# kylegrover/raymarch-algo-compare

Hardware: AMD Instinct MI355X
Metric: Mrays/sec (mean iters/ray alongside), 1920x1080 Mandelbulb/Standard (higher is better)
Workload: dtype f64

## Files before the change

raymarch_algo_compare_amd/csrc/rm_core.h:

```cpp
#pragma once

#include <stdint.h>

#if defined(__HIPCC__)
#include <hip/hip_runtime.h>
#define RM_HD __host__ __device__ __forceinline__
#else
#define RM_HD inline __attribute__((always_inline))
#endif

#include "rm_math.h"

namespace rm {

RM_HD double py_max(double a, double b) { return (b > a) ? b : a; }
RM_HD double py_min(double a, double b) { return (b < a) ? b : a; }

RM_HD double py_mod_pow2(double a, double b)
{
    double m = a - rm_trunc(a / b) * b;
    if (m != 0.0) {
        if (m < 0.0) m += b;
    } else {
        m = 0.0;
// ... 7 lines not shown

RM_HD vec3 v3(double x, double y, double z)
{
    vec3 r;
    r.x = x; r.y = y; r.z = z;
    return r;
}
RM_HD vec3 operator+(vec3 a, vec3 b) { return v3(a.x + b.x, a.y + b.y, a.z + b.z); }
RM_HD vec3 operator-(vec3 a, vec3 b) { return v3(a.x - b.x, a.y - b.y, a.z - b.z); }
RM_HD vec3 operator*(vec3 a, double s) { return v3(a.x * s, a.y * s, a.z * s); }
RM_HD double dot(vec3 a, vec3 b) { return a.x * b.x + a.y * b.y + a.z * b.z; }
RM_HD double pow_half(double x) { return rm_pow(x, 0.5); }
RM_HD double length(vec3 a) { return pow_half(a.x * a.x + a.y * a.y + a.z * a.z); }
RM_HD double pow_half_a(double x) { return rm_pow_half<true>(x); }
RM_HD double length_a(vec3 a) { return pow_half_a(a.x * a.x + a.y * a.y + a.z * a.z); }
RM_HD vec3 normalized(vec3 a)
{
    double l = length(a);
    if (l < 1e-12) return v3(0.0, 0.0, 0.0);
    double inv = 1.0 / l;
    return v3(a.x * inv, a.y * inv, a.z * inv);
}

struct StratParams {
    double omega;
    double ar_omega_min;
    double ar_omega_max;
    double ar_smoothing;
    double ar_growth_rate;
    double ar_decay_rate;
// ... 40 lines not shown
```

raymarch_algo_compare_amd/csrc/rm_kernels.h:

```cpp
#pragma once

#define RM_TABLES_IN_LDS 1

#include <hip/hip_runtime.h>
#include <stdint.h>
#include <type_traits>

#include "rm_camera.h"
#include "rm_capture.h"
#include "rm_scenes.h"
#include "rm_shape.h"
#include "rm_strategies.h"

namespace rm {

constexpr int kHistBins = 544;
constexpr int kStatsHead = 24;
constexpr int kStatsWords = kStatsHead + kHistBins;
constexpr int kQueues = 2;
constexpr int kStatsParts = 64;
constexpr int kStatsBlocks = 1 + kStatsParts;

struct FrameParams {
    CameraParams cam;
// ... 687 lines not shown
    rm_load_tables<Scene>();
    size_t i = (size_t)blockIdx.x * blockDim.x + threadIdx.x;
    if (i >= n) return;
    vec3 o = v3(origins[3 * i], origins[3 * i + 1], origins[3 * i + 2]);
    vec3 d = normalized(v3(dirs[3 * i], dirs[3 * i + 1], dirs[3 * i + 2]));
    Result r = march_one<Scene, Strat>(o, d, cfg);
    hit[i] = (uint8_t)r.hit; t[i] = r.t; iters[i] = r.iters; final_sdf[i] = r.final_sdf;
}

constexpr int kTeam = 3;

struct TeamXch {
    double v[2][2 * kTeam][64];
};

template <class Scene, class PartT>
__device__ __forceinline__ bool team_trip(typename Scene::Eval& ev, bool go, PartT part, int lane, TeamXch& x, int& turn)
{
    double o0 = 0.0, o1 = 0.0;
    if constexpr (std::is_same<PartT, int>::value) {
        if (go) Scene::trip_part(ev, part, o0, o1);
    } else {
        if (go) Scene::template trip_part<PartT::value>(ev, o0, o1);
    }
    double (*buf)[64] = x.v[turn & 1];
    ++turn;
    buf[2 * (int)part][lane] = o0;
    buf[2 * (int)part + 1][lane] = o1;
    __syncthreads();
    bool done = true;
    if (go) done = Scene::trip_join(ev, buf[0][lane], buf[1][lane], buf[2][lane], buf[3][lane], buf[4][lane], buf[5][lane]);
    return done;
}

template <class Scene, class = void>
struct ScenePartLoops : std::false_type {};
template <class Scene>
struct ScenePartLoops<Scene, decltype((void)Scene::kPartLoops)> : std::integral_constant<bool, Scene::kPartLoops> {};

template <class Scene, class = void>
struct SceneShortLastTrip : std::false_type {};
template <class Scene>
struct SceneShortLastTrip<Scene, decltype((void)Scene::kLastTrip)> : std::true_type {};

template <class Scene, int P, class Trip>
__device__ __forceinline__ void team_trips_part(bool& ready, const Trip& trip)
{
    if constexpr (SceneShortLastTrip<Scene>::value) {
#pragma unroll 1
        for (int n = 0; n < Scene::kLastTrip && __any(!ready); ++n) {
            const bool fin = trip(std::integral_constant<int, P>(), !ready);
            if (!ready) ready = fin;
        }
    } else {
        while (__any(!ready)) {
            const bool fin = trip(std::integral_constant<int, P>(), !ready);
            if (!ready) ready = fin;
        }
    }
}
template <class Scene, class Trip>
__device__ __forceinline__ void team_trips(int part, bool& ready, typename Scene::Eval& ev, const Trip& trip)
{
    if constexpr (ScenePartLoops<Scene>::value) {
        part = __builtin_amdgcn_readfirstlane(part);
        if (part == 0) team_trips_part<Scene, 0>(ready, trip);
        else if (part == 1) team_trips_part<Scene, 1>(ready, trip);
        else team_trips_part<Scene, 2>(ready, trip);
        if constexpr (SceneShortLastTrip<Scene>::value) {
            if (__any(!ready)) {
                if (!ready) Scene::trip_last(ev);
                ready = true;
            }
        }
    } else {
        static_assert(!SceneShortLastTrip<Scene>::value, "the short last trip is built into the per-part loops only");
        while (__any(!ready)) {
            const bool fin = trip(part, !ready);
            if (!ready) ready = fin;
        }
    }
}

// ... 13 lines not shown
    const int lane = lane_id();
    const int part = (int)(threadIdx.x >> 6);
    const size_t i = (size_t)blockIdx.x * 64 + (size_t)lane;
    const bool have = i < n;
    vec3 o = v3(0.0, 0.0, 0.0), d = v3(0.0, 0.0, 1.0);
    if (have) {
        o = v3(origins[3 * i], origins[3 * i + 1], origins[3 * i + 2]);
        d = normalized(v3(dirs[3 * i], dirs[3 * i + 1], dirs[3 * i + 2]));
    }
    Strat s;
    bool done = true;
    if (have) done = s.start(cfg);
    typename Scene::Eval ev;
    int turn = 0;
    while (__any(!done)) {
        bool ready = true;
        if (!done) ready = Scene::begin(ev, o + d * s.te);
        team_trips<Scene>(part, ready, ev, [&](auto P, bool go) { return team_trip<Scene>(ev, go, P, lane, xch, turn); });
        if (!done) done = s.step(Scene::value(ev), cfg);
    }
    if (have && part == 0) {
        hit[i] = (uint8_t)s.res.hit; t[i] = s.res.t; iters[i] = s.res.iters; final_sdf[i] = s.res.final_sdf;
    }
    if (busy && threadIdx.x == 0) __hip_atomic_fetch_add(busy, 1ull, __ATOMIC_RELAXED, __HIP_MEMORY_SCOPE_AGENT);
}

template <class Scene, class Strat, bool BATCH>
__global__ __launch_bounds__(64 * kTeam) void resume_team_kernel(const KernelArgs a, const int level)
{
    using Entry = QEntry<Strat>;
    __shared__ TeamXch xch;
    __shared__ unsigned int s_hist[kHistBins];
    __shared__ unsigned int s_base;
// ... 60 lines not shown
                        lane_cfg.full = a.full;
                    } else {
                        camera_ray(a.single.cam, a.width, a.height, x, gy, origin, dir);
                    }
                    active = true;
                }
            }
        }
        if (!__any(active)) {
            if (!more) break;
            continue;
        }

        bool ready = true;
        if (active) ready = Scene::begin(ev, origin + dir * s.te);
        team_trips<Scene>(part, ready, ev, [&](auto P, bool go) { return team_trip<Scene>(ev, go, P, lane, xch, turn); });
        bool park = false;
        if (active) {
            ++nev;
            if (!s.step(Scene::value(ev), cfg)) {
                park = a.suspend_after > 0 && s.i >= a.suspend_after;
            } else {
            active = false;
            if (part == 0) {
                const int it = s.res.iters, h = s.res.hit;
                a.depth[my_gi] = h ? (float)s.res.t : 0.0f;
                a.iters[my_gi] = it;
                a.hit[my_gi] = (uint8_t)h;
                if (raw_out) store_raw(a, my_gi, s.res, nev);
                acc.evals += (unsigned)nev;
                acc.add(it, h);
// ... 113 lines not shown
```

raymarch_algo_compare_amd/csrc/rm_math_atan.h:

```cpp
#pragma once

namespace rm {

struct AtanK {
    static constexpr double hpi = 0x1.921fb54442d18p+0, hpi1 = 0x1.1a62633145c07p-54;
    static constexpr double opi = 0x1.921fb54442d18p+1, opi1 = 0x1.1a62633145c07p-53;
    static constexpr double d3 = -0x1.5555555555555p-2, d5 = 0x1.99999999997fdp-3, d7 = -0x1.24924923f7603p-3,
                            d9 = 0x1.c71c6e5129a3bp-4, d11 = -0x1.7458022b13c25p-4, d13 = 0x1.375f08b31cbcep-4;
    static constexpr double f1 = 0x1.55555555554f9p-3, f2 = 0x1.333333336127dp-4, f3 = 0x1.6db6dae42c0e4p-5,
                            f4 = 0x1.f1c7e04f4ad99p-6, f5 = 0x1.6e442c822d419p-6, f6 = 0x1.292d80f453c72p-6;
    static constexpr double rt0 = 0x1.fffffffecc1ddp-1, rt1 = 0x1.fffffff757304p-2, rt2 = 0x1.800496769c91ap-2,
                            rt3 = 0x1.4006318d1dab9p-2;
    static constexpr double t27 = 0x1p27;
};


RM_MATH_HD double rm_acos_sqrt_band(double x, int m)
{
    typedef AtanK K;
    const double zp = 1.0 - x, zn = x + 1.0;
    double z = ((m > 0) ? zp : zn) * 0.5;
    const int kz = (int)(rm_asuint64(z) >> 32);
    double t = rm_inroot[(kz >> 14) & 0x7f] * rm_asdouble((uint64_t)((1023 + 511 - (kz >> 21)) & 0x7ff) << 52);
    double r = rm_fnma(t * t, z, 1.0);
// ... 6 lines not shown
    double y = rm_fnma(K::t27, c, rm_fma(c, K::t27, c));
    double ty = rm_fma(h, c, y);
    double cc = rm_fnma(y, y, z) / ty;
    double p = rm_fma(z, K::f6, K::f5);
    p = rm_fma(z, p, K::f4);
    p = rm_fma(z, p, K::f3);
    p = rm_fma(z, p, K::f2);
    p = rm_fma(z, p, K::f1);
    double pz = (p * z) * (y + cc);
    const double res_neg = ((K::hpi1 - cc) - pz) + (K::hpi - y);
    const double res_pos = (cc + pz) + y;
    const double res = (m < 0) ? res_neg : res_pos;
    return res + res;
}

RM_MATH_HD double rm_acos_team(double x)
{
    typedef AtanK K;
    const uint64_t bits = rm_asuint64(x);
    const int m = (int)(bits >> 32);
    const int k = m & 0x7fffffff;
    const bool pos = m > 0;
    const double ax = rm_fabs(x);
    const bool in_taylor = k < 0x3fc00000, in_sqrt = k >= 0x3fef0000;
    const bool any_special = rm_band_needed<true>((k < 0x3c880000) | (k >= 0x3ff00000));

    double res = 0.0;
    if (rm_band_needed<true>(!in_taylor & !in_sqrt)) {
        const int r1 = (k >> 15) & 0x1f, r2 = 32 + ((k >> 14) & 0x3f), r3 = 96 + ((k >> 13) & 0x7f);
        int row = (k >= 0x3fd00000) ? r2 : r1;
        row = (k >= 0x3fe00000) ? r3 : row;
// ... 29 lines not shown
    }
    if (rm_band_needed<true>(in_sqrt & (k < 0x3ff00000))) {
        const double res_sqrt = rm_acos_sqrt_band(x, m);
        res = in_sqrt ? res_sqrt : res;
    }
    if (any_special) {
        res = (k < 0x3c880000) ? K::hpi : res;
        const double at_one = pos ? 0.0 : K::opi;
        const bool is_one = (k == 0x3ff00000) & ((uint32_t)bits == 0);
        const double beyond = is_one ? at_one : __builtin_nan("");
        res = (k >= 0x3ff00000) ? beyond : res;
    }
    return res;
}

template <bool U = false>
RM_MATH_HD double rm_acos(double x)
{
    typedef AtanK K;
    if constexpr (U) return rm_acos_team(x);
    const uint64_t bits = rm_asuint64(x);
    const int m = (int)(bits >> 32);
    const int k = m & 0x7fffffff;
    const bool pos = m > 0;
    const double ax = rm_fabs(x);

    double res_taylor = 0.0;
    if (rm_band_needed<U>(k < 0x3fc00000)) {
        const double x2 = x * x;
        double pt = rm_fma(x2, K::f6, K::f5);
        pt = rm_fma(x2, pt, K::f4);
        pt = rm_fma(x2, pt, K::f3);
        pt = rm_fma(x2, pt, K::f2);
        pt = rm_fma(x2, pt, K::f1);
        const double rt = K::hpi - x;
// ... 36 lines not shown
    res = (k >= 0x3ff00000) ? beyond : res;
    return res;
}


RM_MATH_HD double rm_atan_series(double v)
{
    typedef AtanK K;
    double p = rm_fma(v, K::d13, K::d11);
    p = rm_fma(v, p, K::d9);
    p = rm_fma(v, p, K::d7);
    p = rm_fma(v, p, K::d5);
    return rm_fma(v, p, K::d3);
}

RM_MATH_HD double rm_atan2_team(double y, double x)
{
    typedef AtanK K;
    const uint32_t ux = (uint32_t)(rm_asuint64(x) >> 32), uy = (uint32_t)(rm_asuint64(y) >> 32);
    const int de = (int)(uy & 0x7ff00000u) - (int)(ux & 0x7ff00000u);
    const uint32_t lo_e = (1023u - 500u) << 20, span_e = 1000u << 20;
    const bool off_path = rm_band_needed<true>((((ux & 0x7ff00000u) - lo_e) >= span_e) | (((uy & 0x7ff00000u) - lo_e) >= span_e) |
                                               ((uint32_t)(de + (56 << 20)) > (uint32_t)(112 << 20)));

    double ax = rm_fabs(x), ay = rm_fabs(y);
    if (off_path) {
        const double up = ((ax < 0x1p-500) | (ay < 0x1p-500)) ? 0x1p500 : 1.0;
        ax *= up; ay *= up;
        const double dn = ((ax > 0x1p500) | (ay > 0x1p500)) ? 0x1p-500 : 1.0;
        ax *= dn; ay *= dn;
    }
// ... 53 lines not shown
    }
    if (off_path) {
        const bool xneg = (ux & 0x80000000u) != 0;
        const double z_tiny = xpos ? u : K::opi;
        z = (de <= -59768832) ? z_tiny : z;
        z = (de >= 59768832) ? K::hpi : z;
        z = (x == 0.0) ? K::hpi : z;
        const double z_y0 = xneg ? K::opi : 0.0;
        z = (y == 0.0) ? z_y0 : z;
        const bool nonfinite = ((ux & 0x7ff00000u) == 0x7ff00000u) | ((uy & 0x7ff00000u) == 0x7ff00000u);
        z = nonfinite ? __builtin_nan("") : z;
    }
    return __builtin_copysign(z, y);
}

template <bool U = false>
RM_MATH_HD double rm_atan2(double y, double x)
{
    typedef AtanK K;
    if constexpr (U) return rm_atan2_team(y, x);
    const uint32_t ux = (uint32_t)(rm_asuint64(x) >> 32), uy = (uint32_t)(rm_asuint64(y) >> 32);
    const int de = (int)(uy & 0x7ff00000u) - (int)(ux & 0x7ff00000u);

    double ax = rm_fabs(x), ay = rm_fabs(y);
    const double up = ((ax < 0x1p-500) | (ay < 0x1p-500)) ? 0x1p500 : 1.0;
    ax *= up; ay *= up;
    const double dn = ((ax > 0x1p500) | (ay > 0x1p500)) ? 0x1p-500 : 1.0;
    ax *= dn; ay *= dn;

    const bool y_lt_x = ay < ax;
    const double num = y_lt_x ? ay : ax, den = y_lt_x ? ax : ay;
    const double u = num / den;
    const double vq = den * u;
    const double du = ((num - vq) - rm_fma(den, u, -vq)) / den;

// ... 63 lines not shown
```

raymarch_algo_compare_amd/csrc/rm_math_pow.h:

```cpp
#pragma once

#include "rm_tables.h"

namespace rm {

RM_MATH_HD uint64_t rm_asuint64(double x) { return __builtin_bit_cast(uint64_t, x); }
RM_MATH_HD double rm_asdouble(uint64_t u) { return __builtin_bit_cast(double, u); }

RM_MATH_HD double rm_pow_log_inline(uint64_t ix, double* tail)
{
    const double Ln2hi = rm_pow_log_head[0], Ln2lo = rm_pow_log_head[1];
    const double A0 = rm_pow_log_head[2], A1 = rm_pow_log_head[3], A2 = rm_pow_log_head[4],
                 A3 = rm_pow_log_head[5], A4 = rm_pow_log_head[6], A5 = rm_pow_log_head[7],
                 A6 = rm_pow_log_head[8];
    uint64_t tmp = ix - 0x3fe6955500000000ull;
    int i = (int)((tmp >> 45) & 127);
    int k = (int)((int64_t)tmp >> 52);
    uint64_t iz = ix - (tmp & 0xfff0000000000000ull);
    double z = rm_asdouble(iz);
    double kd = (double)k;
    double invc = tab_pow_log(i, 0);
    double logc = tab_pow_log(i, 1);
    double logctail = tab_pow_log(i, 2);

// ... 92 lines not shown
#if defined(__HIP_DEVICE_COMPILE__)
    if constexpr (SPARSE) {
        if (__popcll(__ballot(true)) <= kSparseLanes) {
            bool safe;
            double r = rm_pow_half_guard(x, &safe);
            if (__any(!safe)) {
                const double full = rm_pow(x, 0.5);
                r = safe ? r : full;
            }
            return r;
        }
    }
#endif
    return rm_pow(x, 0.5);
}
RM_MATH_HD void rm_pow2(double x, double ya, double yb, double* ra, double* rb)
{
    double lo;
    double hi = rm_pow_log_inline(rm_pow_norm_bits(x), &lo);
    double ehia = ya * hi, ehib = yb * hi;
    double eloa = rm_fma(ya, lo, rm_fma(hi, ya, -ehia));
    double elob = rm_fma(yb, lo, rm_fma(hi, yb, -ehib));
    *ra = rm_pow_fix_special(x, rm_pow_exp_inline(ehia, eloa));
    *rb = rm_pow_fix_special(x, rm_pow_exp_inline(ehib, elob));
}

}
```

raymarch_algo_compare_amd/csrc/rm_math_trig.h:

```cpp
#pragma once

namespace rm {


struct SinCosK {
    static constexpr double big = 0x1.8p45, toint = 0x1.8p52;
    static constexpr double hpinv = 0x1.45f306dc9c883p-1;
    static constexpr double hp0 = 0x1.921fb54442d18p+0, hp1 = 0x1.1a62633145c07p-54;
    static constexpr double mp1 = 0x1.921fb58000000p+0, mp2 = -0x1.dde973c000000p-27;
    static constexpr double pp3 = -0x1.cb3b398000000p-55, pp4 = -0x1.d747f23e32ed7p-83;
    static constexpr double sn3 = -0x1.5555555555515p-3, sn5 = 0x1.11110e829872fp-7;
    static constexpr double cs2 = 0.5, cs4 = -0x1.5555555555535p-5, cs6 = 0x1.6c16bedd9e239p-10;
    static constexpr double s1 = -0x1.5555555555555p-3, s2 = 0x1.1111111110ecep-7, s3 = -0x1.a01a019db08b8p-13,
                            s4 = 0x1.71de27b9a7ed9p-19, s5 = -0x1.addffc2fcdf59p-26;
};

RM_MATH_HD double rm_fnma(double a, double b, double c) { return rm_fma(-a, b, c); }

template <bool U>
RM_MATH_HD bool rm_band_needed(bool lane_selects)
{
#if defined(__HIP_DEVICE_COMPILE__)
    if constexpr (U) return __any(lane_selects) != 0;
#endif
    (void)lane_selects;
    return true;
}

RM_MATH_HD double rm_taylor_sin(double x, double dx)
{
    typedef SinCosK K;
    double xx = x * x;
    double p = rm_fma(xx, K::s5, K::s4);
    p = rm_fma(xx, p, K::s3);
    p = rm_fma(xx, p, K::s2);
    p = rm_fma(xx, p, K::s1);
    double q = rm_fma(p, x, -(dx * 0.5));
    double t = rm_fma(xx, q, dx);
    return x + t;
}

// ... 27 lines not shown
{
    typedef SinCosK K;
    const double aa = rm_fabs(a);
    const double dx = (a < 0.0) ? -da : da;
    const double u = K::big + aa;
    const double x = (aa - (u - K::big)) + dx;
    const int k = rm_sincos_row(u);
    const double sn = tab_sincos(k, 0), ssn = tab_sincos(k, 1), cs = tab_sincos(k, 2), ccs = tab_sincos(k, 3);
    const double xx = x * x;
    const double s = rm_fma(x * xx, rm_fma(xx, K::sn5, K::sn3), x);
    const double c = xx * rm_fma(xx, rm_fma(xx, K::cs6, K::cs4), K::cs2);
    const double cor = rm_fnma(s, sn, rm_fnma(c, cs, rm_fnma(s, ssn, ccs)));
    return cs + cor;
}

RM_MATH_HD double rm_do_sin_team(double a, double da)
{
    typedef SinCosK K;
    const double aa = rm_fabs(a);
    const double dx = (a <= 0.0) ? -da : da;
    const double u = K::big + aa;
    const double x = aa - (u - K::big);
    const int k = rm_sincos_row(u);
    const double sn = tab_sincos(k, 0), ssn = tab_sincos(k, 1), cs = tab_sincos(k, 2), ccs = tab_sincos(k, 3);
    const double xx = x * x;
    const double s = x + rm_fma(x * xx, rm_fma(xx, K::sn5, K::sn3), dx);
    const double c = rm_fma(x, dx, xx * rm_fma(xx, rm_fma(xx, K::cs6, K::cs4), K::cs2));
    const double cor = rm_fma(s, cs, rm_fnma(c, sn, rm_fma(s, ccs, ssn)));
    double res = __builtin_copysign(sn + cor, a);
    if (rm_band_needed<true>(aa < 0.126)) {
        const double taylor = rm_taylor_sin(a, da);
        res = (aa < 0.126) ? taylor : res;
    }
    return res;
}

RM_MATH_HD void rm_sincos_team(double x, double* sin_out, double* cos_out)
{
    typedef SinCosK K;
    const uint32_t k = (uint32_t)(rm_asuint64(x) >> 32) & 0x7fffffffu;
    const double ax = rm_fabs(x);
    const bool r1 = k < 0x3feb6000u;
    const bool r2 = !r1 & (k < 0x400368fdu);
    const bool any_r2 = rm_band_needed<true>(r2);
    const bool any_edge = rm_band_needed<true>(r2 | (k - 0x3e500000u >= 0x419921fbu - 0x3e500000u));
    const double t = rm_fma(x, K::hpinv, K::toint);
    const double xn = r1 ? 0.0 : (t - K::toint);
    const uint32_t n = r1 ? 0u : (uint32_t)rm_asuint64(t);
    const double y = rm_fnma(xn, K::mp2, rm_fnma(xn, K::mp1, x));
    const double t2 = rm_fnma(xn, K::pp3, y);
    double db = rm_fnma(K::pp3, xn, y - t2);
    const double b = rm_fnma(xn, K::pp4, t2);
    db = db + rm_fnma(xn, K::pp4, t2 - b);

    double aS = b, daS = db, aC = b, daC = db;
    if (any_r2) {
        const double tt = K::hp0 - ax;
        const double a2 = tt + K::hp1;
        const double da2 = (tt - a2) + K::hp1;
        aS = r2 ? a2 : b, daS = r2 ? da2 : db, aC = r2 ? tt : b, daC = r2 ? K::hp1 : db;
    }
    const double dS = rm_do_sin_team(aS, daS);
    const double dC = rm_do_cos(aC, daC);

    const uint32_t m = n + 1u;
    double s = (n & 1u) ? dC : dS;
    s = (n & 2u) ? -s : s;
    double c = (m & 1u) ? dC : dS;
    c = (m & 2u) ? -c : c;
    if (any_edge) {
        const double s2 = __builtin_copysign(dC, x);
        s = r2 ? s2 : s, c = r2 ? dS : c;
        s = (k < 0x3e500000u) ? x : s;
        c = (k < 0x3e400000u) ? 1.0 : c;
        const double bad = __builtin_nan("");
        const bool huge = k >= 0x419921fbu;
        s = huge ? bad : s;
        c = huge ? bad : c;
    }
    *sin_out = s;
    *cos_out = c;
}

template <bool U = false>
RM_MATH_HD void rm_sincos(double x, double* sin_out, double* cos_out)
{
    typedef SinCosK K;
    if constexpr (U) return rm_sincos_team(x, sin_out, cos_out);
    const uint32_t k = (uint32_t)(rm_asuint64(x) >> 32) & 0x7fffffffu;
    const double ax = rm_fabs(x);
    const bool r1 = k < 0x3feb6000u;
    const bool r2 = !r1 & (k < 0x400368fdu);
    const double t = rm_fma(x, K::hpinv, K::toint);
    const double xn = r1 ? 0.0 : (t - K::toint);
    const uint32_t n = r1 ? 0u : (uint32_t)rm_asuint64(t);
    const double y = rm_fnma(xn, K::mp2, rm_fnma(xn, K::mp1, x));
    const double t2 = rm_fnma(xn, K::pp3, y);
    double db = rm_fnma(K::pp3, xn, y - t2);
    const double b = rm_fnma(xn, K::pp4, t2);
    db = db + rm_fnma(xn, K::pp4, t2 - b);
    const double tt = K::hp0 - ax;
    const double a2 = tt + K::hp1;
    const double da2 = (tt - a2) + K::hp1;
// ... 92 lines not shown
```

raymarch_algo_compare_amd/csrc/rm_pipeline.h:

```cpp
#pragma once

#include "rm_kernels.h"

namespace rm {

constexpr int kCtlStride = 16;
constexpr int kCTile = 0;
constexpr int kCReserved = 1;
constexpr int kCTaken = 3;
constexpr int kCFreshDone = 5;
constexpr int kCProdExited = 6;
constexpr int kCLeft = 7;
constexpr int kCLateStarted = 8;
constexpr int kCTeamDone = 9;
constexpr int kCtlWords = 10 * kCtlStride;
__device__ __forceinline__ unsigned long long* ctl(const KernelArgs& a, int k) { return a.ctl + k * kCtlStride; }
constexpr int kWMarkStart = 13;
constexpr int kWMarkFresh = 14;
constexpr int kWMarkProd = 15;
constexpr int kWMarkTiles = 17;
constexpr int kWMarkPush = 18;
constexpr int kWMarkPop = 19;
constexpr int kWLongPushMax = 20;
constexpr int kWLongTeamMax = 21;
// ... 154 lines not shown
        const uint32_t y = pix / (uint32_t)a.width, x = pix - y * (uint32_t)a.width;
        atomicMax(&a.tile_cost[frame * (uint32_t)a.tiles_per_frame + (y / (uint32_t)a.tile_h) * (uint32_t)a.tiles_x + (x >> 6)], it);
    }
}

template <class Scene, class E>
__device__ __forceinline__ auto early_handover(const KernelArgs& a, const E& ev, int i) -> decltype(Scene::eval_trips(ev), bool())
{
    return a.early_handover > 0 && i >= a.early_handover && Scene::eval_trips(ev) >= a.early_trips;
}
template <class Scene>
__device__ __forceinline__ bool early_handover(const KernelArgs&, const NoEval&, int) { return false; }
template <class Scene, class E>
__device__ __forceinline__ bool early_handover(const KernelArgs&, const E&, long) { return false; }

template <class Scene, class Strat, bool BATCH>
__device__ __forceinline__ void pipe_team_role(const KernelArgs& a, const KernelArgs& ar, PipeTeamLds& L, const int part, const int lane)
{
    WaveAcc acc;
    if (a.team_prio >= 3) __builtin_amdgcn_s_setprio(3);
    else if (a.team_prio == 2) __builtin_amdgcn_s_setprio(2);
    else if (a.team_prio == 1) __builtin_amdgcn_s_setprio(1);
    bool active = false;
    uint32_t my_gi = 0;
    uint32_t my_push = 0;
    uint32_t my_pop = 0, nev_pop = 0;
    int nev = 0;
    vec3 origin = v3(0.0, 0.0, 0.0), dir = v3(0.0, 0.0, 0.0);
    MarchCfg lane_cfg = a.single.cfg;
    if constexpr (!BATCH) pin_cfg(lane_cfg);
    const MarchCfg& cfg = lane_cfg;
// ... 66 lines not shown
                        lane_cfg.full = ar.full;
                    } else {
                        camera_ray(ar.single.cam, ar.width, ar.height, x, gy, origin, dir);
                    }
                    active = true;
                }
            } else if (nidle == 64) {
                __builtin_amdgcn_s_sleep(127);
                __builtin_amdgcn_s_sleep(127);
                continue;
            }
        }
        if (!__any(active)) continue;

        ++since_try;
        bool ready = true;
        if (active) ready = Scene::begin(ev, origin + dir * s.te);
        team_trips<Scene>(part, ready, ev, [&](auto P, bool go) { return team_trip<Scene>(ev, go, P, lane, L.xch, turn); });
        const int live = a.trace ? __popcll(__ballot(active)) : 0;
        if (active) {
            ++nev;
            if (s.step(Scene::value(ev), cfg)) {
                active = false;
                if (part == 0) {
                    store_direct(ar, my_gi, s.res, nev, acc, L.hist);
                    if (ar.trace) {
                        const uint32_t k = atomicAdd(&ar.trace[0], 1u);
                        if (k < ar.trace_cap) {
                            uint32_t* const r = ar.trace + 8 + 8 * (size_t)k;
                            r[0] = my_gi; r[1] = (uint32_t)s.res.iters; r[2] = my_push; r[3] = my_pop;
                            r[4] = (uint32_t)(realtime() - ~ld_relaxed(&ar.stats[kWMarkStart]));
                            r[5] = nev_pop; r[6] = (uint32_t)nev; r[7] = (uint32_t)blockIdx.x | ((uint32_t)live << 16);
                        }
// ... 48 lines not shown
    constexpr int kRole[8] = { 0, 1, 2, -1, -1, -1, -1, -1 };
    const int wave_role = !team_wg ? -2 : kRole[wave & 7];
    const bool team_role = team_wg && wave_role >= 0;
    if (team_wg) {
        PipeTeamLds& T = *reinterpret_cast<PipeTeamLds*>(s_role);
        for (int b = threadIdx.x; b < kHistBins; b += blockDim.x) T.hist[b] = 0u;
        if (threadIdx.x == 0) { T.base = T.count = T.queue = T.done = 0u; T.ok_lo = T.ok_hi = 0u; }
        __syncthreads();
    }

    if constexpr (TEAM_ROLE) {
    if (team_wg && wave_role == -1) return;
    if (team_role) {
        const int team = wave_role / kTeam;
        const int part = wave_role % kTeam;
        pipe_team_role<Scene, Strat, BATCH>(a, a, reinterpret_cast<PipeTeamLds*>(s_role)[team], part, lane);
        return;
    }
    }

    PLds& L = *reinterpret_cast<PLds*>(s_role);
    float (*const s_depth)[TILE_PIX] = L.depth[wave];
    uint32_t (*const s_ih)[TILE_PIX] = L.ih[wave];
    const int ntiles = ka.tiles_per_frame * ka.nframes;
    const int team_wgs = TEAM_ROLE ? a.team_wgs : 0;
    int pwave = ((int)blockIdx.x - team_wgs) * kPipeWaves + wave;
    if constexpr (SPLIT) pwave = __builtin_amdgcn_readfirstlane(pwave);
    const int park0 = ka.suspend_after;
    const int park1 = (TEAMS && ka.team_wgs > 0) ? ka.suspend_after2 : 0;
    const bool queues = park0 > 0;
    const bool detach = SPLIT || a.q0_detach != 0;
// ... 369 lines not shown
    if (threadIdx.x == 0) s_args = a;
    pipeline_body<Scene, Strat, TILE_H, INTERLEAVE, BATCH, false, true>(a, s_args);
}

template <class Scene, class Strat, bool BATCH>
__global__ __launch_bounds__(64 * kTeam) void pipeline_team_kernel(const KernelArgs a)
{
    __shared__ PipeTeamLds T;
    __shared__ KernelArgs s_args;
    if (threadIdx.x == 0) s_args = a;
    for (int b = threadIdx.x; b < kHistBins; b += blockDim.x) T.hist[b] = 0u;
    if (threadIdx.x == 0) { T.base = T.count = T.queue = T.done = 0u; T.ok_lo = T.ok_hi = 0u; }
    rm_load_tables<Scene>();
    __syncthreads();
    if (a.marks && threadIdx.x == 0) atomicMax(&a.stats[kWMarkStart], ~realtime());
    pipe_team_role<Scene, Strat, BATCH>(a, s_args, T, (int)(threadIdx.x >> 6), lane_id());
}

}
```

raymarch_algo_compare_amd/csrc/rm_scenes.h:

```cpp
#pragma once

#include "rm_core.h"

namespace rm {

enum : unsigned { TB_POW = 1u, TB_SINCOS = 2u, TB_ACOS = 4u, TB_ATAN = 8u, TB_LOG = 16u };
template <class Scene> struct SceneTables { static constexpr unsigned value = TB_POW; };
template <class Scene> struct SceneIterative { static constexpr bool value = false; };


RM_HD double sd_sphere(vec3 p, double radius) { return length(p) - radius; }

RM_HD double sd_box(vec3 p, vec3 b)
{
    vec3 q = v3(rm_fabs(p.x) - b.x, rm_fabs(p.y) - b.y, rm_fabs(p.z) - b.z);
    double outside = length(v3(py_max(q.x, 0.0), py_max(q.y, 0.0), py_max(q.z, 0.0)));
    double inside = py_min(py_max(q.x, py_max(q.y, q.z)), 0.0);
    return outside + inside;
}

RM_HD double sd_plane(vec3 p, vec3 n, double offset) { return dot(p, n) - offset; }

RM_HD double sd_cylinder(vec3 p, double radius, double half_height)
{
// ... 102 lines not shown
            d = py_max(d, c);
        }
        return d;
    }
};
struct SceneMandelbulb {
    struct Eval {
        vec3 p, z;
        double dr, r;
        int32_t i;
    };
    static RM_HD bool begin(Eval& e, vec3 p)
    {
        e.p = p; e.z = p; e.dr = 1.0; e.i = 0;
        e.r = length_a(p);
        return e.r > 4.0;
    }
    static RM_HD int eval_trips(const Eval& e) { return e.i; }
    static RM_HD bool trip(Eval& e)
    {
        const double power = 8.0;
        const vec3 z = e.z;
        const double r = e.r;
        double theta = rm_acos(py_max(-1.0, py_min(1.0, z.z / py_max(r, 1e-12))));
        double phi = rm_atan2(z.y, z.x);
        double r7, zr;
        rm_pow2(r, power - 1.0, power, &r7, &zr);
        e.dr = r7 * power * e.dr + 1.0;
        theta *= power;
        phi *= power;
// ... 2 lines not shown
        rm_sincos(phi, &sp, &cp);
        e.z = v3(zr * st * cp, zr * st * sp, zr * ct) + e.p;
        if (++e.i >= 8) return true;
        e.r = length_a(e.z);
        return e.r > 4.0;
    }
    static constexpr int kLastTrip = 7;
    static RM_HD void trip_last(Eval& e)
    {
        const double power = 8.0;
        const double r7 = rm_pow(e.r, power - 1.0);
        e.dr = r7 * power * e.dr + 1.0;
        e.i = kLastTrip + 1;
    }
    static constexpr bool kPartLoops = true;
    template <int P>
    static RM_HD void trip_part(const Eval& e, double& o0, double& o1)
    {
        const double power = 8.0;
        if constexpr (P == 0) {
            double theta = rm_acos<true>(py_max(-1.0, py_min(1.0, e.z.z / py_max(e.r, 1e-12))));
            theta *= power;
            rm_sincos<true>(theta, &o0, &o1);
        } else if constexpr (P == 1) {
            double phi = rm_atan2<true>(e.z.y, e.z.x);
            phi *= power;
            rm_sincos<true>(phi, &o0, &o1);
        } else {
            rm_pow2(e.r, power - 1.0, power, &o0, &o1);
        }
    }
    static RM_HD void trip_part(const Eval& e, int part, double& o0, double& o1)
    {
        if (part == 0) trip_part<0>(e, o0, o1);
        else if (part == 1) trip_part<1>(e, o0, o1);
        else trip_part<2>(e, o0, o1);
    }
    static RM_HD bool trip_join(Eval& e, double st, double ct, double sp, double cp, double r7, double zr)
    {
        const double power = 8.0;
        e.dr = r7 * power * e.dr + 1.0;
        e.z = v3(zr * st * cp, zr * st * sp, zr * ct) + e.p;
        if (++e.i >= 8) return true;
        e.r = length_a(e.z);
        return e.r > 4.0;
    }
    static RM_HD double value(const Eval& e)
    {
        return 0.5 * rm_log(py_max(e.r, 1e-12)) * e.r / py_max(e.dr, 1e-12);
    }
    static RM_HD double sdf(vec3 p)
    {
        Eval e;
        bool done = begin(e, p);
#pragma unroll 1
        for (int i = 0; !done; ++i) {
            if (i == kLastTrip) { trip_last(e); break; }
            done = trip(e);
        }
// ... 209 lines not shown
```

Before: 288.8.

## Add common-path fast branches for team math and sparse-wave evaluation

Splits the team acos, atan2 and sincos into a common path that takes a single table branch unless a wave-wide rare check sees lanes needing the Taylor, sqrt or edge bands. It also adds a sparse-wave mode: when few lanes are live, the evaluation uses a different sqrt routine and reads the wave's own trip-part outputs from registers rather than LDS. The aim is to cut divergent band evaluation and exchange overhead in the Mandelbulb team kernels, at the cost of more code paths and template instantiations. The older banded path is kept for the non-flag pipeline role.

```diff
diff --git a/raymarch_algo_compare_amd/csrc/rm_core.h b/raymarch_algo_compare_amd/csrc/rm_core.h
--- a/raymarch_algo_compare_amd/csrc/rm_core.h
+++ b/raymarch_algo_compare_amd/csrc/rm_core.h
@@ -45,6 +45,7 @@
 RM_HD double length(vec3 a) { return pow_half(a.x * a.x + a.y * a.y + a.z * a.z); }
 RM_HD double pow_half_a(double x) { return rm_pow_half<true>(x); }
 RM_HD double length_a(vec3 a) { return pow_half_a(a.x * a.x + a.y * a.y + a.z * a.z); }
+RM_HD double length_a(vec3 a, bool sparse) { return rm_pow_half_sparse(a.x * a.x + a.y * a.y + a.z * a.z, sparse); }
 RM_HD vec3 normalized(vec3 a)
 {
     double l = length(a);
diff --git a/raymarch_algo_compare_amd/csrc/rm_kernels.h b/raymarch_algo_compare_amd/csrc/rm_kernels.h
--- a/raymarch_algo_compare_amd/csrc/rm_kernels.h
+++ b/raymarch_algo_compare_amd/csrc/rm_kernels.h
@@ -725,14 +725,45 @@
     double v[2][2 * kTeam][64];
 };
 
+template <class Scene, class = void>
+struct SceneSparseFlag : std::false_type {};
+template <class Scene>
+struct SceneSparseFlag<Scene, decltype((void)Scene::kSparseFlag)> : std::integral_constant<bool, Scene::kSparseFlag> {};
+__device__ __forceinline__ bool team_sparse(bool live) { return __popcll(__ballot(live)) <= kSparseLanes; }
+template <class Scene, int P, bool SPARSE>
+__device__ __forceinline__ bool team_trip(typename Scene::Eval& ev, bool go, int lane, TeamXch& x, int& turn)
+{
+    double o0 = 0.0, o1 = 0.0;
+    if (go) Scene::template trip_part<P, SPARSE>(ev, o0, o1);
+    double (*buf)[64] = x.v[turn & 1];
+    ++turn;
+    buf[2 * P][lane] = o0;
+    buf[2 * P + 1][lane] = o1;
+    __syncthreads();
+    bool done = true;
+    if (go) {
+        double v[2 * kTeam];
+#pragma unroll
+        for (int k = 0; k < 2 * kTeam; ++k) v[k] = (k == 2 * P) ? o0 : (k == 2 * P + 1) ? o1 : buf[k][lane];
+        done = Scene::trip_join(ev, v[0], v[1], v[2], v[3], v[4], v[5], SPARSE);
+    }
+    return done;
+}
+
+template <class Scene, int P>
+__device__ __forceinline__ void team_trip_part_banded(const typename Scene::Eval& ev, double& o0, double& o1)
+{
+    if constexpr (SceneSparseFlag<Scene>::value) Scene::template trip_part<P, false>(ev, o0, o1);
+    else Scene::template trip_part<P>(ev, o0, o1);
+}
 template <class Scene, class PartT>
-__device__ __forceinline__ bool team_trip(typename Scene::Eval& ev, bool go, PartT part, int lane, TeamXch& x, int& turn)
+__device__ __forceinline__ bool team_trip_banded(typename Scene::Eval& ev, bool go, PartT part, int lane, TeamXch& x, int& turn)
 {
     double o0 = 0.0, o1 = 0.0;
     if constexpr (std::is_same<PartT, int>::value) {
         if (go) Scene::trip_part(ev, part, o0, o1);
     } else {
-        if (go) Scene::template trip_part<PartT::value>(ev, o0, o1);
+        if (go) team_trip_part_banded<Scene, PartT::value>(ev, o0, o1);
     }
     double (*buf)[64] = x.v[turn & 1];
     ++turn;
@@ -754,8 +785,40 @@
 template <class Scene>
 struct SceneShortLastTrip<Scene, decltype((void)Scene::kLastTrip)> : std::true_type {};
 
+template <class Scene, int P, bool SPARSE>
+__device__ __forceinline__ void team_flag_trips(bool& ready, typename Scene::Eval& ev, int lane, TeamXch& x, int& turn)
+{
+#pragma unroll 1
+    for (int n = 0; n < Scene::kLastTrip && __any(!ready); ++n) {
+        const bool fin = team_trip<Scene, P, SPARSE>(ev, !ready, lane, x, turn);
+        if (!ready) ready = fin;
+    }
+}
+template <class Scene, bool SPARSE>
+__device__ __forceinline__ void team_flag_evaluation(int part, bool live, vec3 o, vec3 d, double t, typename Scene::Eval& ev, int lane,
+                                                     TeamXch& x, int& turn)
+{
+    bool ready = true;
+    if (live) ready = Scene::begin(ev, o + d * t, SPARSE);
+    if (part == 0) team_flag_trips<Scene, 0, SPARSE>(ready, ev, lane, x, turn);
+    else if (part == 1) team_flag_trips<Scene, 1, SPARSE>(ready, ev, lane, x, turn);
+    else team_flag_trips<Scene, 2, SPARSE>(ready, ev, lane, x, turn);
+    if (__any(!ready)) {
+        if (!ready) Scene::trip_last(ev);
+    }
+}
+template <class Scene>
+__device__ __forceinline__ void team_evaluate(int part, bool live, vec3 o, vec3 d, double t, typename Scene::Eval& ev, int lane, TeamXch& x,
+                                              int& turn)
+{
+    static_assert(ScenePartLoops<Scene>::value && SceneShortLastTrip<Scene>::value, "built for the Mandelbulb's loops");
+    part = __builtin_amdgcn_readfirstlane(part);
+    if (team_sparse(live)) team_flag_evaluation<Scene, true>(part, live, o, d, t, ev, lane, x, turn);
+    else team_flag_evaluation<Scene, false>(part, live, o, d, t, ev, lane, x, turn);
+}
+
 template <class Scene, int P, class Trip>
-__device__ __forceinline__ void team_trips_part(bool& ready, const Trip& trip)
+__device__ __forceinline__ void team_trips_banded_part(bool& ready, const Trip& trip)
 {
     if constexpr (SceneShortLastTrip<Scene>::value) {
 #pragma unroll 1
@@ -775,9 +838,9 @@
 {
     if constexpr (ScenePartLoops<Scene>::value) {
         part = __builtin_amdgcn_readfirstlane(part);
-        if (part == 0) team_trips_part<Scene, 0>(ready, trip);
-        else if (part == 1) team_trips_part<Scene, 1>(ready, trip);
-        else team_trips_part<Scene, 2>(ready, trip);
+        if (part == 0) team_trips_banded_part<Scene, 0>(ready, trip);
+        else if (part == 1) team_trips_banded_part<Scene, 1>(ready, trip);
+        else team_trips_banded_part<Scene, 2>(ready, trip);
         if constexpr (SceneShortLastTrip<Scene>::value) {
             if (__any(!ready)) {
                 if (!ready) Scene::trip_last(ev);
@@ -821,9 +884,13 @@
     typename Scene::Eval ev;
     int turn = 0;
     while (__any(!done)) {
-        bool ready = true;
-        if (!done) ready = Scene::begin(ev, o + d * s.te);
-        team_trips<Scene>(part, ready, ev, [&](auto P, bool go) { return team_trip<Scene>(ev, go, P, lane, xch, turn); });
+        if constexpr (SceneSparseFlag<Scene>::value) {
+            team_evaluate<Scene>(part, !done, o, d, s.te, ev, lane, xch, turn);
+        } else {
+            bool ready = true;
+            if (!done) ready = Scene::begin(ev, o + d * s.te);
+            team_trips<Scene>(part, ready, ev, [&](auto P, bool go) { return team_trip_banded<Scene>(ev, go, P, lane, xch, turn); });
+        }
         if (!done) done = s.step(Scene::value(ev), cfg);
     }
     if (have && part == 0) {
@@ -914,7 +981,7 @@
 
         bool ready = true;
         if (active) ready = Scene::begin(ev, origin + dir * s.te);
-        team_trips<Scene>(part, ready, ev, [&](auto P, bool go) { return team_trip<Scene>(ev, go, P, lane, xch, turn); });
+        team_trips<Scene>(part, ready, ev, [&](auto P, bool go) { return team_trip_banded<Scene>(ev, go, P, lane, xch, turn); });
         bool park = false;
         if (active) {
             ++nev;
diff --git a/raymarch_algo_compare_amd/csrc/rm_math_atan.h b/raymarch_algo_compare_amd/csrc/rm_math_atan.h
--- a/raymarch_algo_compare_amd/csrc/rm_math_atan.h
+++ b/raymarch_algo_compare_amd/csrc/rm_math_atan.h
@@ -44,7 +44,46 @@
     return res + res;
 }
 
-RM_MATH_HD double rm_acos_team(double x)
+RM_MATH_HD double rm_acos_table_band(int k, double ax, bool pos)
+{
+    typedef AtanK K;
+    const int r1 = (k >> 15) & 0x1f, r2 = 32 + ((k >> 14) & 0x3f), r3 = 96 + ((k >> 13) & 0x7f);
+    int row = (k >= 0x3fd00000) ? r2 : r1;
+    row = (k >= 0x3fe00000) ? r3 : row;
+    row = (row > 215) ? 215 : row;
+    const double* a = rm_asncs + 13 * row;
+    const double a0 = a[0], a1 = a[1], a2 = a[2], a3 = a[3], a4 = a[4], a5 = a[5], a6 = a[6], a7 = a[7], a8 = a[8],
+                 a9 = a[9], a10 = a[10], c0 = a[11], cv = a[12];
+    const double xx = ax - a0;
+    double p = rm_fma(xx, a10, a9);
+    p = rm_fma(xx, p, a8);
+    p = rm_fma(xx, p, a7);
+    p = rm_fma(xx, p, a6);
+    p = rm_fma(xx, p, a5);
+    p = rm_fma(xx, p, a4);
+    p = rm_fma(xx, p, a3);
+    p = rm_fma(xx, p, a2);
+    p = rm_fma(xx * xx, p, c0);
+    const double t = rm_fma(xx, a1, p);
+    const double yb = pos ? (K::hpi - cv) : (cv + K::hpi);
+    const double tb = pos ? (K::hpi1 - t) : (t + K::hpi1);
+    return tb + yb;
+}
+
+RM_MATH_HD double rm_acos_taylor_band(double x)
+{
+    typedef AtanK K;
+    const double x2 = x * x;
+    double pt = rm_fma(x2, K::f6, K::f5);
+    pt = rm_fma(x2, pt, K::f4);
+    pt = rm_fma(x2, pt, K::f3);
+    pt = rm_fma(x2, pt, K::f2);
+    pt = rm_fma(x2, pt, K::f1);
+    const double rt = K::hpi - x;
+    return rt + rm_fnma(pt, x * x2, ((K::hpi - rt) - x) + K::hpi1);
+}
+
+RM_MATH_HD double rm_acos_team_banded(double x)
 {
     typedef AtanK K;
     const uint64_t bits = rm_asuint64(x);
@@ -104,11 +143,45 @@
     return res;
 }
 
+template <bool COMMON = true>
+RM_MATH_HD double rm_acos_team(double x)
+{
+    typedef AtanK K;
+    if constexpr (!COMMON) return rm_acos_team_banded(x);
+    const uint64_t bits = rm_asuint64(x);
+    const int m = (int)(bits >> 32);
+    const int k = m & 0x7fffffff;
+    const bool pos = m > 0;
+    const double ax = rm_fabs(x);
+    const bool in_taylor = k < 0x3fc00000, in_sqrt = k >= 0x3fef0000;
+    if (!RM_UNLIKELY(rm_team_rare(in_taylor | in_sqrt, RM_SITE_ACOS))) return rm_acos_table_band(k, ax, pos);
+
+    const bool any_special = rm_band_needed<true>((k < 0x3c880000) | (k >= 0x3ff00000));
+    double res = 0.0;
+    if (rm_band_needed<true>(!in_taylor & !in_sqrt)) res = rm_acos_table_band(k, ax, pos);
+    if (rm_band_needed<true>(in_taylor)) {
+        const double res_taylor = rm_acos_taylor_band(x);
+        res = in_taylor ? res_taylor : res;
+    }
+    if (rm_band_needed<true>(in_sqrt & (k < 0x3ff00000))) {
+        const double res_sqrt = rm_acos_sqrt_band(x, m);
+        res = in_sqrt ? res_sqrt : res;
+    }
+    if (any_special) {
+        res = (k < 0x3c880000) ? K::hpi : res;
+        const double at_one = pos ? 0.0 : K::opi;
+        const bool is_one = (k == 0x3ff00000) & ((uint32_t)bits == 0);
+        const double beyond = is_one ? at_one : __builtin_nan("");
+        res = (k >= 0x3ff00000) ? beyond : res;
+    }
+    return res;
+}
+
 template <bool U = false>
 RM_MATH_HD double rm_acos(double x)
 {
     typedef AtanK K;
-    if constexpr (U) return rm_acos_team(x);
+    if constexpr (U) return rm_acos_team<true>(x);
     const uint64_t bits = rm_asuint64(x);
     const int m = (int)(bits >> 32);
     const int k = m & 0x7fffffff;
@@ -175,7 +248,105 @@
     return rm_fma(v, p, K::d3);
 }
 
-RM_MATH_HD double rm_atan2_team(double y, double x)
+RM_MATH_HD void rm_atan2_quotient(double ax, double ay, bool* y_lt_x_out, double* u_out, double* du_out)
+{
+    const bool y_lt_x = ay < ax;
+    const double num = y_lt_x ? ay : ax, den = y_lt_x ? ax : ay;
+    const double u = num / den;
+    const double vq = den * u;
+    *du_out = ((num - vq) - rm_fma(den, u, -vq)) / den;
+    *u_out = u;
+    *y_lt_x_out = y_lt_x;
+}
+
+RM_MATH_HD double rm_atan2_series_forms(double u, double du, bool case_i, bool plus, double B, double B1)
+{
+    const double v2 = u * u;
+    const double ser = rm_atan_series(v2);
+    const double uv = u * v2;
+    const double z_is = u + rm_fma(uv, ser, du);
+    const double su = plus ? u : -u, sdu = plus ? du : -du;
+    const double zz_s = uv * ser;
+    const double t2 = B + su;
+    const double cor = (B - t2) + su;
+    const double z_os = (((cor + B1) + sdu) + (plus ? zz_s : -zz_s)) + t2;
+    return case_i ? z_is : z_os;
+}
+
+RM_MATH_HD const double* rm_atan2_table_row(double u)
+{
+    int i = (int)(rm_fma(u, 256.0, 0x1p52) - 0x1p52) - 16;
+    i = (i < 0) ? 0 : ((i > 240) ? 240 : i);
+    return rm_cij + 7 * i;
+}
+
+RM_MATH_HD double rm_atan2_table_i(double t3, double du, double c1, double c2, double c3, double c4, double c5, double c6)
+{
+    const double vi = du + t3;
+    const double dv = (rm_fabs(t3) > rm_fabs(du)) ? ((t3 - vi) + du) : ((du - vi) + t3);
+    double pi_ = rm_fma(vi, c6, c5);
+    pi_ = rm_fma(vi, pi_, c4);
+    pi_ = rm_fma(vi, pi_, c3);
+    pi_ = (vi * vi) * pi_;
+    pi_ = rm_fma(dv, c2, pi_);
+    return rm_fma(vi, c2, pi_) + c1;
+}
+
+RM_MATH_HD double rm_atan2_table_o(double t3, double du, bool plus, double B, double B1, double c1, double c2, double c3, double c4,
+                                   double c5, double c6)
+{
+    const double vo = t3 + du;
+    double po = rm_fma(vo, c6, c5);
+    po = rm_fma(vo, po, c4);
+    po = rm_fma(vo, po, c3);
+    po = rm_fma(vo, po, c2);
+    return (B + (plus ? c1 : -c1)) + rm_fma(plus ? vo : -vo, po, B1);
+}
+
+RM_MATH_HD double rm_atan2_team_forms(double u, double du, bool case_i, bool plus, double B, double B1)
+{
+    const bool small = u < 0.0625;
+    double z = 0.0;
+    if (rm_band_needed<true>(small)) z = rm_atan2_series_forms(u, du, case_i, plus, B, B1);
+    if (rm_band_needed<true>(!small)) {
+        const double* c = rm_atan2_table_row(u);
+        const double c0 = c[0], c1 = c[1], c2 = c[2], c3 = c[3], c4 = c[4], c5 = c[5], c6 = c[6];
+        const double t3 = u - c0;
+        if (rm_band_needed<true>(!small & case_i)) {
+            const double z_it = rm_atan2_table_i(t3, du, c1, c2, c3, c4, c5, c6);
+            z = (!small & case_i) ? z_it : z;
+        }
+        if (rm_band_needed<true>(!small & !case_i)) {
+            const double z_ot = rm_atan2_table_o(t3, du, plus, B, B1, c1, c2, c3, c4, c5, c6);
+            z = (!small & !case_i) ? z_ot : z;
+        }
+    }
+    return z;
+}
+
+RM_MATH_HD void rm_atan2_rescale(double* ax, double* ay)
+{
+    const double up = ((*ax < 0x1p-500) | (*ay < 0x1p-500)) ? 0x1p500 : 1.0;
+    *ax *= up; *ay *= up;
+    const double dn = ((*ax > 0x1p500) | (*ay > 0x1p500)) ? 0x1p-500 : 1.0;
+    *ax *= dn; *ay *= dn;
+}
+
+RM_MATH_HD double rm_atan2_special_ladder(double y, double x, uint32_t ux, uint32_t uy, int de, bool xpos, double u, double z)
+{
+    typedef AtanK K;
+    const bool xneg = (ux & 0x80000000u) != 0;
+    const double z_tiny = xpos ? u : K::opi;
+    z = (de <= -59768832) ? z_tiny : z;
+    z = (de >= 59768832) ? K::hpi : z;
+    z = (x == 0.0) ? K::hpi : z;
+    const double z_y0 = xneg ? K::opi : 0.0;
+    z = (y == 0.0) ? z_y0 : z;
+    const bool nonfinite = ((ux & 0x7ff00000u) == 0x7ff00000u) | ((uy & 0x7ff00000u) == 0x7ff00000u);
+    return nonfinite ? __builtin_nan("") : z;
+}
+
+RM_MATH_HD double rm_atan2_team_banded(double y, double x)
 {
     typedef AtanK K;
     const uint32_t ux = (uint32_t)(rm_asuint64(x) >> 32), uy = (uint32_t)(rm_asuint64(y) >> 32);
@@ -259,11 +430,50 @@
     return __builtin_copysign(z, y);
 }
 
+template <bool COMMON = true>
+RM_MATH_HD double rm_atan2_team(double y, double x)
+{
+    typedef AtanK K;
+    if constexpr (!COMMON) return rm_atan2_team_banded(y, x);
+    const uint32_t ux = (uint32_t)(rm_asuint64(x) >> 32), uy = (uint32_t)(rm_asuint64(y) >> 32);
+    const int de = (int)(uy & 0x7ff00000u) - (int)(ux & 0x7ff00000u);
+    const uint32_t lo_e = (1023u - 500u) << 20, span_e = 1000u << 20;
+    const bool off_path = (((ux & 0x7ff00000u) - lo_e) >= span_e) | (((uy & 0x7ff00000u) - lo_e) >= span_e) |
+                          ((uint32_t)(de + (56 << 20)) > (uint32_t)(112 << 20));
+    const bool xpos = x > 0.0;
+    double ax = rm_fabs(x), ay = rm_fabs(y);
+    bool y_lt_x;
+    double u, du, z;
+    if (RM_UNLIKELY(rm_team_rare(off_path, RM_SITE_ATAN2_ENTRY))) {
+        rm_atan2_rescale(&ax, &ay);
+        rm_atan2_quotient(ax, ay, &y_lt_x, &u, &du);
+        const bool case_i = xpos & y_lt_x;
+        const bool case_iv = !xpos & !(ax < ay);
+        const bool plus = !xpos & (ax < ay);
+        const double B = case_iv ? K::opi : K::hpi, B1 = case_iv ? K::opi1 : K::hpi1;
+        z = rm_atan2_team_forms(u, du, case_i, plus, B, B1);
+        z = rm_atan2_special_ladder(y, x, ux, uy, de, xpos, u, z);
+    } else {
+        rm_atan2_quotient(ax, ay, &y_lt_x, &u, &du);
+        const bool case_i = xpos & y_lt_x;
+        const bool case_iv = !xpos & !(ax < ay);
+        const bool plus = !xpos & (ax < ay);
+        const double B = case_iv ? K::opi : K::hpi, B1 = case_iv ? K::opi1 : K::hpi1;
+        if (RM_UNLIKELY(rm_team_rare((u < 0.0625) | case_i, RM_SITE_ATAN2_FORM))) {
+            z = rm_atan2_team_forms(u, du, case_i, plus, B, B1);
+        } else {
+            const double* c = rm_atan2_table_row(u);
+            z = rm_atan2_table_o(u - c[0], du, plus, B, B1, c[1], c[2], c[3], c[4], c[5], c[6]);
+        }
+    }
+    return __builtin_copysign(z, y);
+}
+
 template <bool U = false>
 RM_MATH_HD double rm_atan2(double y, double x)
 {
     typedef AtanK K;
-    if constexpr (U) return rm_atan2_team(y, x);
+    if constexpr (U) return rm_atan2_team<true>(y, x);
     const uint32_t ux = (uint32_t)(rm_asuint64(x) >> 32), uy = (uint32_t)(rm_asuint64(y) >> 32);
     const int de = (int)(uy & 0x7ff00000u) - (int)(ux & 0x7ff00000u);
 
diff --git a/raymarch_algo_compare_amd/csrc/rm_math_pow.h b/raymarch_algo_compare_amd/csrc/rm_math_pow.h
--- a/raymarch_algo_compare_amd/csrc/rm_math_pow.h
+++ b/raymarch_algo_compare_amd/csrc/rm_math_pow.h
@@ -130,6 +130,24 @@
 #endif
     return rm_pow(x, 0.5);
 }
+RM_MATH_HD double rm_pow_half_sparse(double x, bool sparse)
+{
+    if (__builtin_expect(sparse, 1)) {
+        bool safe;
+        double r = rm_pow_half_guard(x, &safe);
+#if defined(__HIP_DEVICE_COMPILE__)
+        const bool any_unsafe = __any(!safe) != 0;
+#else
+        const bool any_unsafe = !safe;
+#endif
+        if (__builtin_expect(any_unsafe, 0)) {
+            const double full = rm_pow(x, 0.5);
+            r = safe ? r : full;
+        }
+        return r;
+    }
+    return rm_pow(x, 0.5);
+}
 RM_MATH_HD void rm_pow2(double x, double ya, double yb, double* ra, double* rb)
 {
     double lo;
diff --git a/raymarch_algo_compare_amd/csrc/rm_math_trig.h b/raymarch_algo_compare_amd/csrc/rm_math_trig.h
--- a/raymarch_algo_compare_amd/csrc/rm_math_trig.h
+++ b/raymarch_algo_compare_amd/csrc/rm_math_trig.h
@@ -25,6 +25,20 @@
 #endif
     (void)lane_selects;
     return true;
+}
+
+#define RM_UNLIKELY(c) __builtin_expect(!!(c), 0)
+enum { RM_SITE_ACOS = 0, RM_SITE_SINCOS = 1, RM_SITE_DO_SIN = 2, RM_SITE_ATAN2_ENTRY = 3, RM_SITE_ATAN2_FORM = 4 };
+RM_MATH_HD bool rm_team_rare(bool lane_rare, int site)
+{
+    (void)site;
+#if defined(__HIP_DEVICE_COMPILE__)
+    return __any(lane_rare) != 0;
+#elif defined(RM_TEAM_PATH_FORCE)
+    return RM_TEAM_PATH_FORCE(lane_rare, site);
+#else
+    return lane_rare;
+#endif
 }
 
 RM_MATH_HD double rm_taylor_sin(double x, double dx)
@@ -82,7 +96,28 @@
     return cs + cor;
 }
 
-RM_MATH_HD double rm_do_sin_team(double a, double da)
+RM_MATH_HD double rm_do_sin_table(double a, double da)
+{
+    typedef SinCosK K;
+    const double aa = rm_fabs(a);
+    const double dx = (a <= 0.0) ? -da : da;
+    const double u = K::big + aa;
+    const double x = aa - (u - K::big);
+    const int k = rm_sincos_row(u);
+    const double sn = tab_sincos(k, 0), ssn = tab_sincos(k, 1), cs = tab_sincos(k, 2), ccs = tab_sincos(k, 3);
+    const double xx = x * x;
+    const double s = x + rm_fma(x * xx, rm_fma(xx, K::sn5, K::sn3), dx);
+    const double c = rm_fma(x, dx, xx * rm_fma(xx, rm_fma(xx, K::cs6, K::cs4), K::cs2));
+    const double cor = rm_fma(s, cs, rm_fnma(c, sn, rm_fma(s, ccs, ssn)));
+    return __builtin_copysign(sn + cor, a);
+}
+
+RM_MATH_HD double rm_do_sin_taylor_into(double a, double da, bool in_taylor, double res)
+{
+    const double taylor = rm_taylor_sin(a, da);
+    return in_taylor ? taylor : res;
+}
+RM_MATH_HD double rm_do_sin_team_banded(double a, double da)
 {
     typedef SinCosK K;
     const double aa = rm_fabs(a);
@@ -103,7 +138,63 @@
     return res;
 }
 
-RM_MATH_HD void rm_sincos_team(double x, double* sin_out, double* cos_out)
+template <bool COMMON = true>
+RM_MATH_HD double rm_do_sin_team(double a, double da)
+{
+    if constexpr (!COMMON) return rm_do_sin_team_banded(a, da);
+    const bool in_taylor = rm_fabs(a) < 0.126;
+    double res = rm_do_sin_table(a, da);
+    if (RM_UNLIKELY(rm_team_rare(in_taylor, RM_SITE_DO_SIN))) res = rm_do_sin_taylor_into(a, da, in_taylor, res);
+    return res;
+}
+
+RM_MATH_HD void rm_sincos_reduce(double x, bool r1, double* b_out, double* db_out, uint32_t* n_out)
+{
+    typedef SinCosK K;
+    const double t = rm_fma(x, K::hpinv, K::toint);
+    const double xn = r1 ? 0.0 : (t - K::toint);
+    const uint32_t n = r1 ? 0u : (uint32_t)rm_asuint64(t);
+    const double y = rm_fnma(xn, K::mp2, rm_fnma(xn, K::mp1, x));
+    const double t2 = rm_fnma(xn, K::pp3, y);
+    double db = rm_fnma(K::pp3, xn, y - t2);
+    const double b = rm_fnma(xn, K::pp4, t2);
+    db = db + rm_fnma(xn, K::pp4, t2 - b);
+    *b_out = b; *db_out = db; *n_out = n;
+}
+
+RM_MATH_HD void rm_sincos_route(uint32_t n, double dS, double dC, double* s_out, double* c_out)
+{
+    const uint32_t m = n + 1u;
+    double s = (n & 1u) ? dC : dS;
+    s = (n & 2u) ? -s : s;
+    double c = (m & 1u) ? dC : dS;
+    c = (m & 2u) ? -c : c;
+    *s_out = s; *c_out = c;
+}
+
+RM_MATH_HD void rm_sincos_r2_inputs(double ax, bool r2, double b, double db, double* aS, double* daS, double* aC, double* daC)
+{
+    typedef SinCosK K;
+    const double tt = K::hp0 - ax;
+    const double a2 = tt + K::hp1;
+    const double da2 = (tt - a2) + K::hp1;
+    *aS = r2 ? a2 : b, *daS = r2 ? da2 : db, *aC = r2 ? tt : b, *daC = r2 ? K::hp1 : db;
+}
+
+RM_MATH_HD void rm_sincos_edge_outputs(double x, uint32_t k, bool r2, double dS, double dC, double* s_io, double* c_io)
+{
+    double s = *s_io, c = *c_io;
+    const double s2 = __builtin_copysign(dC, x);
+    s = r2 ? s2 : s, c = r2 ? dS : c;
+    s = (k < 0x3e500000u) ? x : s;
+    c = (k < 0x3e400000u) ? 1.0 : c;
+    const double bad = __builtin_nan("");
+    const bool huge = k >= 0x419921fbu;
+    *s_io = huge ? bad : s;
+    *c_io = huge ? bad : c;
+}
+
+RM_MATH_HD void rm_sincos_team_banded(double x, double* sin_out, double* cos_out)
 {
     typedef SinCosK K;
     const uint32_t k = (uint32_t)(rm_asuint64(x) >> 32) & 0x7fffffffu;
@@ -128,7 +219,7 @@
         const double da2 = (tt - a2) + K::hp1;
         aS = r2 ? a2 : b, daS = r2 ? da2 : db, aC = r2 ? tt : b, daC = r2 ? K::hp1 : db;
     }
-    const double dS = rm_do_sin_team(aS, daS);
+    const double dS = rm_do_sin_team_banded(aS, daS);
     const double dC = rm_do_cos(aC, daC);
 
     const uint32_t m = n + 1u;
@@ -150,11 +241,39 @@
     *cos_out = c;
 }
 
+template <bool COMMON = true>
+RM_MATH_HD void rm_sincos_team(double x, double* sin_out, double* cos_out)
+{
+    if constexpr (!COMMON) return rm_sincos_team_banded(x, sin_out, cos_out);
+    const uint32_t k = (uint32_t)(rm_asuint64(x) >> 32) & 0x7fffffffu;
+    const bool r1 = k < 0x3feb6000u;
+    const bool r2 = !r1 & (k < 0x400368fdu);
+    const bool edge = r2 | (k - 0x3e500000u >= 0x419921fbu - 0x3e500000u);
+    double b, db, s, c;
+    uint32_t n;
+    if (RM_UNLIKELY(rm_team_rare(edge, RM_SITE_SINCOS))) {
+        double aS, daS, aC, daC;
+        rm_sincos_reduce(x, r1, &b, &db, &n);
+        rm_sincos_r2_inputs(rm_fabs(x), r2, b, db, &aS, &daS, &aC, &daC);
+        const double dS = rm_do_sin_team<true>(aS, daS);
+        const double dC = rm_do_cos(aC, daC);
+        rm_sincos_route(n, dS, dC, &s, &c);
+        rm_sincos_edge_outputs(x, k, r2, dS, dC, &s, &c);
+    } else {
+        rm_sincos_reduce(x, r1, &b, &db, &n);
+        const double dS = rm_do_sin_team<true>(b, db);
+        const double dC = rm_do_cos(b, db);
+        rm_sincos_route(n, dS, dC, &s, &c);
+    }
+    *sin_out = s;
+    *cos_out = c;
+}
+
 template <bool U = false>
 RM_MATH_HD void rm_sincos(double x, double* sin_out, double* cos_out)
 {
     typedef SinCosK K;
-    if constexpr (U) return rm_sincos_team(x, sin_out, cos_out);
+    if constexpr (U) return rm_sincos_team<true>(x, sin_out, cos_out);
     const uint32_t k = (uint32_t)(rm_asuint64(x) >> 32) & 0x7fffffffu;
     const double ax = rm_fabs(x);
     const bool r1 = k < 0x3feb6000u;
diff --git a/raymarch_algo_compare_amd/csrc/rm_pipeline.h b/raymarch_algo_compare_amd/csrc/rm_pipeline.h
--- a/raymarch_algo_compare_amd/csrc/rm_pipeline.h
+++ b/raymarch_algo_compare_amd/csrc/rm_pipeline.h
@@ -192,7 +192,7 @@
 template <class Scene, class E>
 __device__ __forceinline__ bool early_handover(const KernelArgs&, const E&, long) { return false; }
 
-template <class Scene, class Strat, bool BATCH>
+template <class Scene, class Strat, bool BATCH, bool BY_FLAG>
 __device__ __forceinline__ void pipe_team_role(const KernelArgs& a, const KernelArgs& ar, PipeTeamLds& L, const int part, const int lane)
 {
     WaveAcc acc;
@@ -289,9 +289,13 @@
         if (!__any(active)) continue;
 
         ++since_try;
-        bool ready = true;
-        if (active) ready = Scene::begin(ev, origin + dir * s.te);
-        team_trips<Scene>(part, ready, ev, [&](auto P, bool go) { return team_trip<Scene>(ev, go, P, lane, L.xch, turn); });
+        if constexpr (BY_FLAG && SceneSparseFlag<Scene>::value) {
+            team_evaluate<Scene>(part, active, origin, dir, s.te, ev, lane, L.xch, turn);
+        } else {
+            bool ready = true;
+            if (active) ready = Scene::begin(ev, origin + dir * s.te);
+            team_trips<Scene>(part, ready, ev, [&](auto P, bool go) { return team_trip_banded<Scene>(ev, go, P, lane, L.xch, turn); });
+        }
         const int live = a.trace ? __popcll(__ballot(active)) : 0;
         if (active) {
             ++nev;
@@ -370,7 +374,7 @@
     if (team_role) {
         const int team = wave_role / kTeam;
         const int part = wave_role % kTeam;
-        pipe_team_role<Scene, Strat, BATCH>(a, a, reinterpret_cast<PipeTeamLds*>(s_role)[team], part, lane);
+        pipe_team_role<Scene, Strat, BATCH, false>(a, a, reinterpret_cast<PipeTeamLds*>(s_role)[team], part, lane);
         return;
     }
     }
@@ -770,7 +774,7 @@
     rm_load_tables<Scene>();
     __syncthreads();
     if (a.marks && threadIdx.x == 0) atomicMax(&a.stats[kWMarkStart], ~realtime());
-    pipe_team_role<Scene, Strat, BATCH>(a, s_args, T, (int)(threadIdx.x >> 6), lane_id());
-}
-
-}
+    pipe_team_role<Scene, Strat, BATCH, true>(a, s_args, T, (int)(threadIdx.x >> 6), lane_id());
+}
+
+}
diff --git a/raymarch_algo_compare_amd/csrc/rm_scenes.h b/raymarch_algo_compare_amd/csrc/rm_scenes.h
--- a/raymarch_algo_compare_amd/csrc/rm_scenes.h
+++ b/raymarch_algo_compare_amd/csrc/rm_scenes.h
@@ -140,6 +140,13 @@
     {
         e.p = p; e.z = p; e.dr = 1.0; e.i = 0;
         e.r = length_a(p);
+        return e.r > 4.0;
+    }
+    static constexpr bool kSparseFlag = true;
+    static RM_HD bool begin(Eval& e, vec3 p, bool sparse)
+    {
+        e.p = p; e.z = p; e.dr = 1.0; e.i = 0;
+        e.r = length_a(p, sparse);
         return e.r > 4.0;
     }
     static RM_HD int eval_trips(const Eval& e) { return e.i; }
@@ -172,18 +179,18 @@
         e.i = kLastTrip + 1;
     }
     static constexpr bool kPartLoops = true;
-    template <int P>
+    template <int P, bool COMMON = true>
     static RM_HD void trip_part(const Eval& e, double& o0, double& o1)
     {
         const double power = 8.0;
         if constexpr (P == 0) {
-            double theta = rm_acos<true>(py_max(-1.0, py_min(1.0, e.z.z / py_max(e.r, 1e-12))));
+            double theta = rm_acos_team<COMMON>(py_max(-1.0, py_min(1.0, e.z.z / py_max(e.r, 1e-12))));
             theta *= power;
-            rm_sincos<true>(theta, &o0, &o1);
+            rm_sincos_team<COMMON>(theta, &o0, &o1);
         } else if constexpr (P == 1) {
-            double phi = rm_atan2<true>(e.z.y, e.z.x);
+            double phi = rm_atan2_team<COMMON>(e.z.y, e.z.x);
             phi *= power;
-            rm_sincos<true>(phi, &o0, &o1);
+            rm_sincos_team<COMMON>(phi, &o0, &o1);
         } else {
             rm_pow2(e.r, power - 1.0, power, &o0, &o1);
         }
@@ -201,6 +208,15 @@
         e.z = v3(zr * st * cp, zr * st * sp, zr * ct) + e.p;
         if (++e.i >= 8) return true;
         e.r = length_a(e.z);
+        return e.r > 4.0;
+    }
+    static RM_HD bool trip_join(Eval& e, double st, double ct, double sp, double cp, double r7, double zr, bool sparse)
+    {
+        const double power = 8.0;
+        e.dr = r7 * power * e.dr + 1.0;
+        e.z = v3(zr * st * cp, zr * st * sp, zr * ct) + e.p;
+        if (++e.i >= 8) return true;
+        e.r = length_a(e.z, sparse);
         return e.r > 4.0;
     }
     static RM_HD double value(const Eval& e)
```

Result: faster. 298.9, median of 6 (+3.5%).
